# chrhansk/sleqp

Measured on AMD Instinct MI355X. Metric: KKT factor+solve/sec (numeric refactor + 1 solve with device-controlled refinement, inputs resident in HBM), higher is better.
Workload: dtype f64; 1 GPU; banded_n1e5_m5e4; n=100000, m=50000, N=150000, nnz_J=1000000, nnz_tril_K=1100000, nnz_L=11646539, nnz_L_stored=12226637, supernodes=569, etree_levels=10, refine_steps=1, hip_graphs=5, solves_per_factor=1, parallelism=single

## Files before the change

include/hipfact.h:

```cpp
#ifndef HIPFACT_H
#define HIPFACT_H

#include <stddef.h>
#include <stdint.h>

#ifdef __cplusplus
extern "C" {
#endif

#define HIPFACT_VERSION "0.1.0"

enum
{
  HIPFACT_OK         = 0,
  HIPFACT_EINVAL     = -1,
  HIPFACT_EDEVICE    = -2,
  HIPFACT_ESINGULAR  = -3,
  HIPFACT_ENOMEM     = -4,
  HIPFACT_ESTATE     = -5,
  HIPFACT_EINTERNAL  = -6
};

typedef struct hipfact_handle hipfact_handle;

// ... 151 lines not shown
  HIPFACT_LSQR_TIME      = 3,
  HIPFACT_LSQR_ZERO      = 4
};

typedef struct hipfact_lsqr_info
{
  double time_limit;
  int iterations;
  int status;
  int timed_out;
  double phi_bar;
} hipfact_lsqr_info;

int hipfact_lsqr_solve(hipfact_handle* h, const hipfact_lsqr_op* op, const double* rhs, double rel_tol,
                       double trust_radius, double eps, int max_iter, double* step, hipfact_lsqr_info* info);

int hipfact_tridiag_tr(int k, const double* delta, const double* gamma, double gamma0, double radius, double* h,
                       double* lambda);


int hipfact_set_option(hipfact_handle* h, const char* name, double value);

int hipfact_get_info(const hipfact_handle* h, const char* name, double* value);

int hipfact_debug_copy(hipfact_handle* h, const char* name, void* out, size_t bytes);

int hipfact_debug_pool_selftest(int callers, int rounds);

int hipfact_debug_place_rows(int m, const int* Ar_ptr, long long fill_bytes, int classes, long long* bounds, int* classes_out,
                             int* grid_out, int* blocks);
int hipfact_debug_place_items(int nfronts, const int* counts, int classes, int* order, int* lost);

int hipfact_debug_multi_slices(int u, int slice_rows, int* tile_bounds , int cap);

int hipfact_debug_extra_rule(int nblocks, int npasses, const double* dn, const double* zn, int pass_cap, int* applied,
                             int* status, double* ferr, double* rho);
int hipfact_debug_multi_extra_schedule(int ncols, int nblocks, int npasses, const double* dn, const double* zn,
                                       int pass_cap, unsigned int* open_mask, hipfact_extra_info* info);
int hipfact_debug_condest_dense(int N, const double* A, long long ld, hipfact_cond_info* info,
                                double* witness , int* history , int cap);
int hipfact_debug_condest_recorded(int N, int nrecords, const double* records, hipfact_cond_info* info);
enum {
  HIPFACT_CADENCE_FACTOR = 0,
  HIPFACT_CADENCE_SOLVE = 1,
  HIPFACT_CADENCE_VERDICT = 2,
  HIPFACT_CADENCE_JUDGE = 3,
  HIPFACT_CADENCE_RESET = 4,
  HIPFACT_CADENCE_SET_STEPS = 5,
  HIPFACT_CADENCE_SET_CHECK_EVERY = 6,
  HIPFACT_CADENCE_SET_CHECK_BACKOFF = 7,
  HIPFACT_CADENCE_SAVE = 8,
  HIPFACT_CADENCE_RESTORE = 9,
  HIPFACT_CADENCE_DEVICE_RESIDUAL = 10,
  HIPFACT_CADENCE_EVENT_WIDTH = 8,
  HIPFACT_CADENCE_ROW_WIDTH = 20
};
int hipfact_debug_refine_cadence(const int* knobs , int nevents, const double* events, long long* rows);
double hipfact_debug_dd_residual(int nterms, const double* k, const double* z, double b, int lanes);


typedef struct hipfact_plan hipfact_plan;
int hipfact_plan_create(int N, const int* colptr, const int* rowidx, const double* vals ,
                        hipfact_plan** out);
void hipfact_plan_free(hipfact_plan** plan);
const char* hipfact_plan_error(const hipfact_plan* plan);
int hipfact_plan_array(const hipfact_plan* plan, const char* name, const void** data, int64_t* len,
// ... 9 lines not shown
```

sleqp_amd/_lib.py:

```python
from __future__ import annotations

import ctypes as C
import os

_HERE = os.path.dirname(os.path.abspath(__file__))
LIB_PATH = os.environ.get("HIPFACT_LIBRARY") or os.path.join(_HERE, "csrc", "libhipfact.so")

HIPFACT_OK = 0
ERRORS = {
    -1: "HIPFACT_EINVAL",
    -2: "HIPFACT_EDEVICE",
    -3: "HIPFACT_ESINGULAR",
    -4: "HIPFACT_ENOMEM",
    -5: "HIPFACT_ESTATE",
    -6: "HIPFACT_EINTERNAL",
}

SYMBOLS = [
    "hipfact_create", "hipfact_free", "hipfact_retain", "hipfact_last_error", "hipfact_last_warning", "hipfact_set_matrix", "hipfact_solve_sparse",
    "hipfact_solve_dense", "hipfact_solution", "hipfact_solution_view", "hipfact_condition", "hipfact_refactor_device",
    "hipfact_solve_device", "hipfact_solve_device_multi", "hipfact_solve_multi",
    "hipfact_condition_estimate", "hipfact_debug_condest_dense", "hipfact_debug_condest_recorded",
    "hipfact_solve_device_extra", "hipfact_solve_extra", "hipfact_residual_device", "hipfact_debug_extra_rule", "hipfact_debug_dd_residual",
    "hipfact_solve_device_multi_extra", "hipfact_solve_multi_extra", "hipfact_residual_device_multi", "hipfact_debug_multi_extra_schedule",
    "hipfact_solution_device", "hipfact_synchronize", "hipfact_check", "hipfact_stream",
    "hipfact_assemble_kkt", "hipfact_reduced_matrix", "hipfact_spmat_create", "hipfact_spmat_update_values", "hipfact_spmat_free",
    "hipfact_spmat_mult_vec", "hipfact_spmat_mult_vec_trans", "hipfact_spmat_mult_vec_sym",
    "hipfact_spmat_mult_device", "hipfact_steihaug_solve", "hipfact_tr_solve", "hipfact_tr_solve_ex", "hipfact_lsqr_solve", "hipfact_tridiag_tr", "hipfact_set_option", "hipfact_get_info", "hipfact_debug_copy", "hipfact_debug_pool_selftest",
    "hipfact_debug_place_rows", "hipfact_debug_place_items", "hipfact_debug_multi_slices", "hipfact_debug_refine_cadence", "hipfact_plan_create",
    "hipfact_plan_free", "hipfact_plan_error", "hipfact_plan_array", "hipfact_plan_scalar",
]

_lib = None


class HipfactError(RuntimeError):
    def __init__(self, code: int, message: str):
        super().__init__(f"{ERRORS.get(code, code)}: {message}")
        self.code = code


def load() -> C.CDLL:
    global _lib
    if _lib is not None:
        return _lib
    if not os.path.exists(LIB_PATH):
        raise ImportError(
            f"{LIB_PATH} not found: build the HIP extension first "
            "(python -c 'import __graft_entry__ as g; g.build()' or make -C sleqp_amd/csrc)")
    lib = C.CDLL(LIB_PATH)
    vp, ci, cd = C.c_void_p, C.c_int, C.c_double
    lib.hipfact_create.argtypes = [C.POINTER(vp), ci]
    lib.hipfact_free.argtypes = [C.POINTER(vp)]
    lib.hipfact_retain.argtypes = [vp]
    lib.hipfact_last_error.argtypes = [vp]
    lib.hipfact_last_error.restype = C.c_char_p
    lib.hipfact_last_warning.argtypes = [vp]
    lib.hipfact_last_warning.restype = C.c_char_p
    lib.hipfact_set_matrix.argtypes = [vp, ci, vp, vp, vp]
    lib.hipfact_solve_sparse.argtypes = [vp, ci, ci, vp, vp]
    lib.hipfact_solve_dense.argtypes = [vp, vp]
    lib.hipfact_solution.argtypes = [vp, vp, ci, ci]
# ... 17 lines not shown
        lib.hipfact_residual_device_multi.argtypes = [vp, ci, vp, ll, vp, ll, vp, ll, ci]
        lib.hipfact_debug_multi_extra_schedule.argtypes = [ci, ci, ci, vp, vp, ci, vp, vp]
    if hasattr(lib, "hipfact_condition_estimate"):
        lib.hipfact_condition_estimate.argtypes = [vp, ci, vp, vp]
        lib.hipfact_debug_condest_dense.argtypes = [ci, vp, C.c_longlong, vp, vp, vp, ci]
        lib.hipfact_debug_condest_recorded.argtypes = [ci, ci, vp, vp]
    lib.hipfact_solution_device.argtypes = [vp, C.POINTER(vp)]
    lib.hipfact_synchronize.argtypes = [vp]
    lib.hipfact_check.argtypes = [vp]
    lib.hipfact_stream.argtypes = [vp, C.POINTER(vp)]
    lib.hipfact_assemble_kkt.argtypes = [vp, ci, ci, vp, vp, vp, vp, vp, ci, C.POINTER(ci), vp, vp, vp]
    lib.hipfact_reduced_matrix.argtypes = [vp, C.POINTER(ci), vp, vp, vp]
    lib.hipfact_spmat_create.argtypes = [vp, ci, ci, vp, vp, vp, C.POINTER(vp)]
    lib.hipfact_spmat_update_values.argtypes = [vp, vp]
    lib.hipfact_spmat_free.argtypes = [C.POINTER(vp)]
    lib.hipfact_spmat_mult_vec.argtypes = [vp, vp, vp]
    lib.hipfact_spmat_mult_vec_trans.argtypes = [vp, vp, vp]
    lib.hipfact_spmat_mult_vec_sym.argtypes = [vp, vp, vp]
    lib.hipfact_spmat_mult_device.argtypes = [vp, ci, vp, vp]
    lib.hipfact_steihaug_solve.argtypes = [vp, vp, vp, cd, cd, ci, vp, C.POINTER(cd), C.POINTER(ci)]
    lib.hipfact_tr_solve.argtypes = [vp, ci, vp, vp, vp, vp, cd, cd, ci, vp, C.POINTER(cd), C.POINTER(ci)]
    lib.hipfact_tr_solve_ex.argtypes = [vp, ci, vp, vp, vp, vp, cd, cd, ci, vp, C.POINTER(cd), C.POINTER(ci), vp]
    lib.hipfact_lsqr_solve.argtypes = [vp, vp, vp, cd, cd, cd, ci, vp, vp]
    lib.hipfact_tridiag_tr.argtypes = [ci, vp, vp, cd, cd, vp, C.POINTER(cd)]
    lib.hipfact_set_option.argtypes = [vp, C.c_char_p, cd]
    lib.hipfact_debug_copy.argtypes = [vp, C.c_char_p, vp, C.c_size_t]
    lib.hipfact_debug_pool_selftest.argtypes = [ci, ci]
    lib.hipfact_get_info.argtypes = [vp, C.c_char_p, C.POINTER(cd)]
    if hasattr(lib, "hipfact_debug_place_items"):
        lib.hipfact_debug_place_rows.argtypes = [ci, vp, C.c_longlong, ci, vp, C.POINTER(ci), C.POINTER(ci), vp]
        lib.hipfact_debug_place_items.argtypes = [ci, vp, ci, vp, vp]
    if hasattr(lib, "hipfact_debug_multi_slices"):
        lib.hipfact_debug_multi_slices.argtypes = [ci, ci, vp, ci]
    if hasattr(lib, "hipfact_debug_refine_cadence"):
        lib.hipfact_debug_refine_cadence.argtypes = [vp, ci, vp, vp]
    lib.hipfact_plan_create.argtypes = [ci, vp, vp, vp, C.POINTER(vp)]
    lib.hipfact_plan_free.argtypes = [C.POINTER(vp)]
    lib.hipfact_plan_error.argtypes = [vp]
    lib.hipfact_plan_error.restype = C.c_char_p
    lib.hipfact_plan_array.argtypes = [vp, C.c_char_p, C.POINTER(vp), C.POINTER(C.c_int64), C.POINTER(ci)]
    lib.hipfact_plan_scalar.argtypes = [vp, C.c_char_p, C.POINTER(cd)]
    for name in SYMBOLS:
        if not hasattr(lib, name) and not os.environ.get("HIPFACT_LIBRARY"):
            raise ImportError(f"{LIB_PATH} lacks {name}: rebuild it (make -C sleqp_amd/csrc)")
    lib.hipfact_plan_free.restype = None
    _lib = lib
    return lib


def kernel_sources_sha16() -> str:
    import glob
    import hashlib

    d = os.path.join(os.path.dirname(os.path.abspath(__file__)), "csrc")
    h = hashlib.sha256()
    for name in sorted(glob.glob(os.path.join(d, "*.hip")) + glob.glob(os.path.join(d, "*.inc")) + glob.glob(os.path.join(d, "*.h"))):
        h.update(os.path.basename(name).encode())
        h.update(open(name, "rb").read())
    return h.hexdigest()[:16]
```

sleqp_amd/csrc/abi_options.inc:

```
enum OptionEffect {
  FX_NONE,
  FX_GRAPHS,
  FX_GRAPHS_IF_CHANGED,
  FX_PLANS,
  FX_PLANS_IF_CHANGED,
};
struct OptionRow {
  const char* name;
  const char* env;
  OptionEffect effect;
  int (*set)(hipfact_handle* h, double v);
  const char* doc;
};
#define OPT_STORE(field, conv)                 \
  [](hipfact_handle* h, double v) -> int {     \
    const auto x = (conv);                     \
    const bool changed = h->field != x;        \
    h->field = x;                              \
    return changed;                            \
  }
static const OptionRow kOptions[] = {
    {"refine_steps", "HIPFACT_REFINE", FX_GRAPHS,
     [](hipfact_handle* h, double v) -> int {
       h->refine_steps = std::max(0, (int)v);
// ... 135 lines not shown
     },
     "1: K is analysed exactly as given - no row dictionary, unit rows of active bounds stay in the structure (what hipfact_reduced_matrix needs)"},
    {"assemble_superset", nullptr, FX_NONE, OPT_STORE(assemble_superset, v != 0.0),
     "0: hipfact_assemble_kkt analyses every working set on its own rows (no superset plan)"},
    {"plan_cache", nullptr, FX_NONE,
     [](hipfact_handle* h, double v) -> int {
       h->plan_cache_max = std::max(0, (int)v);
       while ((int)h->cache.size() > h->plan_cache_max) h->cache.pop_back();
       return 1;
     },
     "inactive plan states kept (LRU); 0: one pattern at a time"},
    {"profile", nullptr, FX_NONE,
     [](hipfact_handle* h, double v) -> int {
       if (h->prof.on) prof_collect(h);
       if (v < 0)
         for (int c = 0; c < PC_COUNT; ++c) h->prof.ms[c] = 0, h->prof.max_ms[c] = 0, h->prof.cnt[c] = 0;
       h->prof.tagged.clear();
       h->prof.on = v > 0;
       return 1;
     },
     "event-time every kernel class; value < 0 resets the counters"},
    {"ordering", nullptr, FX_PLANS, OPT_STORE(prm.ordering, (int)v),
     "0 nested dissection + AMD leaves (default), 1 AMD on the whole graph, 2 natural"},
    {"max_children", nullptr, FX_PLANS, OPT_STORE(prm.max_children, (int)v),
     "relaxed amalgamation keeps fronts at this many children (default 4 = what the pull extend-add takes in one block)"},
    {"force_generic", nullptr, FX_PLANS, OPT_STORE(prm.force_generic, v != 0.0),
     "1: no saddle-point structure detection, static 1 x 1 pivots on K as given (symmetric positive definite input: the PSD shim)"},
    {"dense_mode", nullptr, FX_PLANS, OPT_STORE(prm.dense_mode, std::min(2, std::max(0, (int)v))),
     "1: late elimination inside the tree (default), 2: low-rank correction, 0: off"},
    {nullptr, "HIPFACT_DATAFLOW_RETRY", FX_NONE, OPT_STORE(df_retry_every, std::max(0, (int)v)), nullptr},
    {nullptr, "HIPFACT_CHECK_LAUNCHES", FX_NONE, OPT_STORE(check_launches, v != 0.0), nullptr},
    {nullptr, "HIPFACT_SOL_SPLIT", FX_NONE, OPT_STORE(sol_split, v != 0.0), nullptr},
    {nullptr, "HIPFACT_IDX64", FX_NONE, OPT_STORE(idx64, v != 0.0), nullptr},
    {nullptr, "HIPFACT_XCD_CLASSES", FX_NONE, OPT_STORE(xcd_classes, std::max(1, std::min(XCD_CLASSES_MAX, (int)v))), nullptr},
    {nullptr, "HIPFACT_RESID_FROM_X", FX_NONE, OPT_STORE(resid_from_x, std::max(0, std::min(3, (int)v))), nullptr},
};
#undef OPT_STORE

static void options_from_environment(hipfact_handle* h) {
  for (const OptionRow& row : kOptions)
    if (const char* s = row.env ? getenv(row.env) : nullptr) (void)row.set(h, (double)atoi(s));
}

int hipfact_set_option(hipfact_handle* h, const char* name, double value) {
  if (!h || !name) return HIPFACT_EINVAL;
  {
    bool known = false;
    const int rc = multi_set_option(h, name, value, known);
    if (known) return rc;
  }
  {
    bool known = false;
    const int rc = condest_set_option(h, name, value, known);
    if (known) return rc;
  }
  for (const OptionRow& row : kOptions) {
    if (!row.name || strcmp(name, row.name)) continue;
    const int changed = row.set(h, value);
    if (changed < 0) return changed;
    if (row.effect == FX_GRAPHS || (row.effect == FX_GRAPHS_IF_CHANGED && changed)) drop_graphs(h);
    if (row.effect == FX_PLANS || (row.effect == FX_PLANS_IF_CHANGED && changed)) invalidate_plans(h);
    return HIPFACT_OK;
  }
  h->error = std::string("unknown option: ") + name;
  return HIPFACT_EINVAL;
}

int hipfact_debug_copy(hipfact_handle* h, const char* name, void* out, size_t bytes) {
  int rc = enter(h);
  if (rc) return rc;
  if (!name || !out) return HIPFACT_EINVAL;
  auto host_copy = [&](const auto& v) {
    if (bytes > v.size() * sizeof(v[0])) {
      h->error = "hipfact_debug_copy: unknown buffer or size";
      return HIPFACT_EINVAL;
    }
    if (bytes) memcpy(out, v.data(), bytes);
    return HIPFACT_OK;
  };
  const Plan& P = h->plan;
  if (!strcmp(name, "perm")) return host_copy(P.perm);
  if (!strcmp(name, "sn_c0")) return host_copy(P.sn_c0);
  if (!strcmp(name, "sn_r")) return host_copy(P.sn_r);
  if (!strcmp(name, "sn_rowptr")) return host_copy(P.sn_rowptr);
  if (!strcmp(name, "sn_rows")) return host_copy(P.sn_rows);
  if (!strcmp(name, "sn_Loff")) return host_copy(P.sn_Loff);
  if (!strcmp(name, "late_cols")) return host_copy(P.late_cols);
  if (!strcmp(name, "sn_level")) return host_copy(P.sn_level);
  if (!strcmp(name, "dense_cols")) return host_copy(P.dense_cols);
  if (!strcmp(name, "cond_history")) return host_copy(h->cond_history);
  const DevBuf* b = nullptr;
  if (!strcmp(name, "L")) b = &h->d_L;
  else if (!strcmp(name, "U")) b = &h->d_U;
  else if (!strcmp(name, "SPf")) b = &h->d_SPf;
  else if (!strcmp(name, "sitems")) b = &h->d_sitems;
  else if (!strcmp(name, "y")) b = &h->d_y;
  else if (!strcmp(name, "xhat")) b = &h->d_xhat;
  else if (!strcmp(name, "ysol")) b = &h->d_ysol;
  else if (!strcmp(name, "uvec")) b = &h->d_uvec;
  else if (!strcmp(name, "dscale")) b = &h->d_dscale;
  else if (!strcmp(name, "Kval")) b = &h->d_Kval;
  else if (!strcmp(name, "res")) b = &h->d_res;
  else if (!strcmp(name, "norms")) b = &h->d_norms;
  else if (!strcmp(name, "mY")) b = &h->d_mY;
  if (!strcmp(name, "cond_d")) {
    const size_t N = (size_t)h->N_ext, off = (2 * COND_T + 3) * N * sizeof(double);
    if (!h->d_cblk.p || bytes > N * sizeof(double)) {
      h->error = "hipfact_debug_copy: unknown buffer or size";
      return HIPFACT_EINVAL;
    }
    HCHECK(h, hipStreamSynchronize(h->stream));
    HCHECK(h, hipMemcpy(out, h->d_cblk.as<char>() + off, bytes, hipMemcpyDeviceToHost));
    return HIPFACT_OK;
  }
  if (!b || !b->p || bytes > b->bytes) {
    h->error = "hipfact_debug_copy: unknown buffer or size";
    return HIPFACT_EINVAL;
  }
  HCHECK(h, hipStreamSynchronize(h->stream));
  HCHECK(h, hipMemcpy(out, b->p, bytes, hipMemcpyDeviceToHost));
  return HIPFACT_OK;
}

int hipfact_debug_place_rows(int m, const int* Ar_ptr, long long fill_bytes, int classes, long long* bounds, int* classes_out,
                             int* grid_out, int* blocks) {
  if (m < 0 || (m > 0 && !Ar_ptr) || fill_bytes < 0 || classes < 1 || classes > XCD_CLASSES_MAX || !bounds || !classes_out ||
      !grid_out || !blocks)
    return HIPFACT_EINVAL;
  ClassBounds cb;
  *grid_out = place_rows(m, Ar_ptr, (size_t)fill_bytes, classes, cb);
  *classes_out = cb.C;
  for (int g = 0; g <= cb.C; ++g) bounds[g] = cb.b[g];
  for (int g = 0; g < cb.C; ++g) class_row_blocks(cb, g, FB / RL, blocks[2 * g], blocks[2 * g + 1]);
  return HIPFACT_OK;
}
int hipfact_debug_place_items(int nfronts, const int* counts, int classes, int* order, int* lost) {
  if (nfronts < 0 || (nfronts > 0 && !counts) || classes < 1 || classes > XCD_CLASSES_MAX) return HIPFACT_EINVAL;
  long long total = 0;
  for (int f = 0; f < nfronts; ++f) {
    if (counts[f] < 0) return HIPFACT_EINVAL;
    total += counts[f];
  }
  if (total >= (1LL << 31) || (total > 0 && (!order || !lost))) return HIPFACT_EINVAL;
  std::vector<int> o, l;
  deal_items(std::vector<int>(counts, counts + nfronts), classes, o, &l);
  for (size_t i = 0; i < o.size(); ++i) {
    order[i] = o[i];
    lost[i] = l[i];
  }
  return HIPFACT_OK;
}

int hipfact_debug_multi_slices(int u, int slice_rows, int* tile_bounds, int cap) {
  if (u < 0 || !multi_slice_rows_valid(slice_rows)) return HIPFACT_EINVAL;
  const int ns = multi_nslice(u, slice_rows);
  if (tile_bounds && ns <= cap)
    for (int k = 0; k <= ns; ++k) tile_bounds[k] = multi_slice_tile(u, ns, k);
  return ns;
}

int hipfact_debug_refine_cadence(const int* knobs, int nevents, const double* events, long long* rows) {
  using namespace hipfact;
  if (!knobs || nevents < 0 || (nevents > 0 && (!events || !rows))) return HIPFACT_EINVAL;
  for (int q = 0; q < 7; ++q)
    if (knobs[q] < 0 || ((q == 1 || q >= 5) && knobs[q] > 1) || (q >= 2 && q <= 4 && knobs[q] < 1)) return HIPFACT_EINVAL;
  CadenceKnobs k{knobs[0], knobs[1] != 0, knobs[2], knobs[3], knobs[4], knobs[5] != 0, knobs[6] != 0};
  FactorCadence f;
  PlanCadence p;
  SolveCadence s;
  LiveCadence l;
  Cadence cad{f, p, s, l};
  SavedCadence saved{};
  bool have_saved = false;
  for (int e = 0; e < nevents; ++e) {
    const double* ev = events + (size_t)e * HIPFACT_CADENCE_EVENT_WIDTH;
    for (int q = 0; q < 6; ++q)
      if (!(std::fabs(ev[q]) < (double)(1 << 30)) || ev[q] != std::floor(ev[q])) return HIPFACT_EINVAL;
    const int kind = (int)ev[0], flag = (int)ev[1];
    const CtlPeek c{(int)ev[2], (int)ev[3], (int)ev[4], (int)ev[5], ev[6], ev[7]};
    const bool yes_no = flag == 0 || flag == 1;
    SolveDecision d{false, false, false, 0, 0};
    switch (kind) {
      case HIPFACT_CADENCE_FACTOR:
// ... 117 lines not shown
  INFO("nlevels", P.nlevels) INFO("nprod", P.nprod) INFO("L_bytes", P.L_size * 8.0) INFO("U_bytes", P.U_size * 8.0)
  INFO("analysis_s", P.t_total) INFO("order_s", P.t_order) INFO("symbolic_s", P.t_symbolic)
  INFO("num_perturbed", h->num_perturbed) INFO("static_pivot_runs", h->static_pivot_runs) INFO("static_pivot_shift", h->reg_delta)
  INFO("num_zero_pivots", h->info_host[INFO_ZERO_PIVOT]) INFO("num_neg_pivots", h->info_host[INFO_NEG_PIVOT])
  INFO("cache_hits", h->cache_hits) INFO("plan_swaps", h->plan_swaps) INFO("plans_cached", h->cache.size())
  INFO("no_dataflow", h->no_dataflow) INFO("dataflow_fallbacks", h->dataflow_fallbacks) INFO("turn_waits", (double)h->turn_waits) INFO("dataflow_rearmed", h->dataflow_rearmed) INFO("fused_solve", h->fused_solve) INFO("spanel_folded", h->sp_folded) INFO("solve_items", h->n_sitems) INFO("chain_levels_fused", [&] { int c = 0; for (const LevelInfo& li : h->levels) c += li.mini_cnt > 0; return c; }()) INFO("solve_panel_bytes", h->sp_bytes) INFO("spf_bytes", (double)h->d_SPf.bytes) INFO("sitem_bytes", (double)sizeof(SolveItem)) INFO("N_internal", P.N) INFO("maps_on", h->maps_on) INFO("m_struct", h->m_struct) INFO("analyses", h->analyses) INFO("num_factor", h->num_factor) INFO("cg_device_runs", h->cg_device_runs) INFO("cg_device_fallbacks", h->cg_device_fallbacks) INFO("lz_device_runs", h->lz_device_runs) INFO("lz_device_fallbacks", h->lz_device_fallbacks) INFO("lz_device_iterations", h->lz_device_iterations) INFO("lsqr_runs", h->lsqr_runs) INFO("lsqr_iters", h->lsqr_iters) INFO("dense_columns", h->nd) INFO("late_columns", P.n_late) INFO("late_rows", P.n_late_rows) INFO("m_rows", P.saddle ? P.my : P.m) INFO("vtable_rows", h->vj->rows()) INFO("vtable_retries", h->vtable_retries) INFO("dense_fallbacks", h->dense_fallbacks) INFO("dense_probes", h->dense_probes) INFO("top_block_cols", h->tb_nT) INFO("top_block_below", h->tb_nfb) INFO("top_block_levels", h->tb_levels) INFO("top_block_items", h->tb_ntf) INFO("top_block_builds", h->tb_builds) INFO("top_block_active", h->tb_valid) INFO("superset_vtable", h->superset_vtable) INFO("exact_pattern", h->exact_pattern) INFO("spmv_stream", h->spmv_stream)
  INFO("boundary_fast", h->boundary_fast) INFO("bd_count", h->bd_count) INFO("bd_stage_us", h->bd_stage_us) INFO("bd_queue_us", h->bd_queue_us) INFO("bd_rhs_us", h->bd_rhs_us) INFO("bd_device_us", h->bd_device_us) INFO("bd_d2h_us", h->bd_d2h_us) INFO("bd_wait_us", h->bd_wait_us) INFO("bd_copyout_us", h->bd_copyout_us)
  INFO("multi_solves", h->multi_solves) INFO("multi_cols", h->multi_cols) INFO("multi_blocks", h->multi_blocks)
  INFO("multi_passes", h->multi_passes) INFO("multi_single_cols", h->multi_single_cols) INFO("multi_failed_col", h->multi_failed_col)
  INFO("multi_sliced_fronts", h->mitems_for < 0 ? 0 : h->n_mcut) INFO("multi_slice_items", h->mitems_for < 0 ? 0 : h->n_mslices) INFO("multi_slice_rows", h->multi_slice_rows)
  INFO("cond_estimates", h->cond_estimates) INFO("cond_blocks", h->cond_blocks) INFO("cond_last", h->cond_last) INFO("condition_estimate", h->condition_estimate)
  INFO("extra_solves", h->extra_solves) INFO("extra_passes", h->extra_passes) INFO("extra_last_status", h->extra_last_status)
  INFO("extra_multi_solves", h->extra_multi_solves) INFO("extra_multi_cols", h->extra_multi_cols) INFO("extra_multi_passes", h->extra_multi_passes)
  INFO("num_solve", h->num_solve) INFO("num_refined", h->solve_cad.num_refined) INFO("refine_adaptive", h->refine_adaptive)
  INFO("num_passes", h->solve_cad.num_passes) INFO("last_omega", h->last_ctl.omega) INFO("last_iters", h->last_ctl.iters)
  INFO("last_status", h->last_ctl.status) INFO("last_tol", h->last_ctl.tol) INFO("kappa_est", h->last_ctl.kappa)
  INFO("refine_inline", h->factor_cad.refine_inline) INFO("refine_tol", h->refine_tol) INFO("equilibrate", h->equilibrate)
  INFO("factor_top_level", h->ftop_level) INFO("factor_top_count", h->ftop_count) INFO("solve_timeouts", h->h_info.p ? h->h_info.as<int>()[INFO_TIMEOUT] : 0)
  INFO("top_level", 1 << 30)
  INFO("use_graph", h->use_graph) INFO("num_graphs", h->graphs.size()) INFO("max_r", P.max_r) INFO("max_w", P.max_w) INFO("refine_steps", h->refine_steps)
  INFO("schur_flops_max_level", h->schur_flops_max)
  INFO("chain_pairs", h->n_pairs)
  INFO("xupd_fused", h->xupd_fused ? 1 : 0)
  INFO("rhs_in_tree", h->last_rhs_in_tree) INFO("xupd_in_tree", h->last_xupd_in_tree) INFO("xupd_blocks_launched", h->last_xupd_blocks)
  INFO("solve_sliced_fronts", h->n_sliced) INFO("solve_resorted_levels", h->n_resorted) INFO("tree_solve", tree_solve(h))
  INFO("refine_check_every", h->refine_check_every) INFO("refine_check_interval", h->solve_cad.check_interval_now) INFO("num_checked", h->solve_cad.num_checked)
  INFO("device", h->device) INFO("nnzM", P.Mi.size()) INFO("nnzA", P.Ar_src.size())
  INFO("rows_total", P.sn_rows.size()) INFO("ent_fused", h->ent_fused) INFO("ent_split", h->ent_split)
  INFO("rows_fused", h->rows_fused) INFO("rows_split", h->rows_split)
  INFO("long_row_segments", h->n_rseg) INFO("row_scale_blocks", row_scale_in_sequence(h) ? h->rs_grid : 0)
  INFO("arena_fill_bytes", arena_fill_bytes(P))
  INFO("resid_blocks", resid_blocks(P)) INFO("resid_from_x", resid_from_x(h)) INFO("resid_queued_from_x", h->resid_queued_from_x) INFO("resid_queued_full", h->resid_queued_full)
  INFO("xcd_classes", h->xcd_classes) INFO("dealt_multi_item_fronts", h->dealt_multi) INFO("long_prod_segments", h->n_lprod)
  INFO("long_col_segments", h->n_cseg) INFO("idx32", h->idx32) INFO("prod_packed", h->prod_packed)
  INFO("active_bounds", h->maps_on ? h->n_bounds : 0)
  INFO("values_in_place",
       h->have_plan && (!h->from_jacobian || (virtual_current(h) && h->vj->identity))) INFO("inactive_rows", h->maps_on ? h->n_inactive : 0)
#undef INFO
  return HIPFACT_EINVAL;
}
```

sleqp_amd/csrc/hipfact.hip:

```cpp
#include <hip/hip_runtime.h>

#include <dlfcn.h>

#include <algorithm>
#include <atomic>
#include <chrono>
#include <cmath>
#include <cstdio>
#include <cstdlib>
#include <cstring>
#include <memory>
#include <new>
#include <string>
#include <condition_variable>
#include <functional>
#include <mutex>
#include <thread>
#include <unordered_map>
#include <vector>

#include "../../include/hipfact.h"
#include "device_types.h"
#include "plan.h"
#include "tridiag_tr.h"

#include "kernel_types.h"
#include "kernels_decl.h"
#include "xcd_place.h"
#include "multi_slices.h"
#include "refine_cadence.h"
#include "condest_rule.h"
#include "dd_arith.h"

#include "runtime_types.inc"
#include "runtime_plan.inc"
#include "runtime_queue.inc"
#include "runtime_multi.inc"
#include "runtime_extra.inc"
#include "runtime_multi_extra.inc"
#include "runtime_condest.inc"

extern "C" {
#include "abi_core.inc"
#include "abi_multi.inc"
#include "abi_extra.inc"
#include "abi_multi_extra.inc"
#include "abi_condest.inc"
#include "abi_working_set.inc"
#include "abi_krylov.inc"
#include "abi_options.inc"
}
```

sleqp_amd/csrc/kernels_factor.hip:

```cpp
#include <hip/hip_runtime.h>

#include "device_types.h"
#include "kernel_types.h"

namespace hipfact {
#include "kernels_common.inc"
#include "kernels_mvals.inc"
#include "kernels_front_pivot.inc"
#include "kernels_front_update.inc"
#include "kernels_front_fused.inc"
#include "kernels_solve_panels.inc"
#include "kernels_factor_top.inc"
}

namespace hipfact {
#define INST_MVALS(IDX, PK)                                                                                          \
  template __global__ void k_mvals_prod<IDX, PK>(long long, const IDX*, const int*, const int*, const IDX*, const double*, \
                                                double*, int, const LongProd*,                                       \
                                                double*, unsigned int*);
INST_MVALS(unsigned int, true)
INST_MVALS(unsigned int, false)
INST_MVALS(long long, true)
INST_MVALS(long long, false)
#undef INST_MVALS
#define INST_FRONT(CH)                                                                                              \
  template __global__ void k_front_pivot<CH>(const FrontItem*, double*, double*, int*, const int*, const int*,     \
                                             const PullDesc*, int);                                                 \
  template __global__ void k_front_panel<CH>(const FrontItem*, double*, double*, const int*, const int*,           \
                                             const PullDesc*, int);                                                 \
  template __global__ void k_front_schur<CH>(const FrontItem*, double*, double*, const int*, const int*,           \
                                             const PullDesc*, int);
INST_FRONT(true)
INST_FRONT(false)
#undef INST_FRONT
}

// ... 12 lines not shown
```

sleqp_amd/csrc/kernels_front_update.inc:

```
template <bool X_IN_LDS, bool RECIP = false>
__device__ __forceinline__ void dev_panel_solve(const FrontCtx& c, int blk, int blk_stride, const PullCtx& pc,
                                                const int* invl) {
  const int wave = threadIdx.x >> 6;
  const int RB = 16 * (blockDim.x >> 6);
  for (int R0 = c.w + RB * blk + 16 * wave; R0 < c.r; R0 += RB * blk_stride) {
    double pv[8][4];
    int cis[MAXCH];
    dev_panel_rows_load(c, R0, pc, pv, cis);
    dev_panel_rows_finish<X_IN_LDS, RECIP>(c, R0, pc, invl, pv, cis);
  }
}

constexpr int KC = 32;
constexpr int SCB = 64;
__device__ __forceinline__ void schur_tile_gather(const PullCtx& pc, const int* invs, int i0, int j0, int li, int lk,
                                                  double (&uv)[2][2][4]) {
#pragma unroll
  for (int ch = 0; ch < MAXCH; ++ch)
    if (ch < pc.n) {
      const double* __restrict__ Uc = pc.Uc[ch];
      const int uc = pc.uc[ch];
      const int* iv = invs + 128 * ch;
      int ci[2], cj[2][4];
#pragma unroll
// ... 354 lines not shown
      J = t - a * (a + 1) / 2;
    } else {
      I = ntc + (t - head) / ntc;
      J = (t - head) % ntc;
    }
    ij = (int)((I << 16) | J);
  } else if (compact) {
    const long long nt = (c.u + 63) / 64;
    long long t = blockIdx.x, jb = 0;
    for (;; ++jb) {
      const long long j0 = jb * SCB, bw = min((long long)SCB, nt - j0), rows = nt - j0;
      const long long cnt = bw * (bw + 1) / 2 + (rows - bw) * bw;
      if (t < cnt) break;
      t -= cnt;
    }
    const long long j0 = jb * SCB, bw = min((long long)SCB, nt - j0), head = bw * (bw + 1) / 2;
    long long I, J;
    if (t < head) {
      long long a = (long long)((sqrt(8.0 * (double)t + 1.0) - 1.0) * 0.5);
      while (a * (a + 1) / 2 > t) --a;
      while ((a + 1) * (a + 2) / 2 <= t) ++a;
      I = j0 + a;
      J = j0 + (t - a * (a + 1) / 2);
    } else {
      I = j0 + bw + (t - head) / bw;
      J = j0 + (t - head) % bw;
    }
    ij = (int)((I << 16) | J);
  }
  dev_schur_tile<false, CHAIN>(c, c.A, c.A + 64 * KC, ij >> 16, ij & 0xffff, S.nchild == 0, pc, threadIdx.x, nullptr, 0,
                               nullptr, PullMore{more, U, inv, rel});
}


__global__ __launch_bounds__(FB, 3) void k_front_schur_pair(const FrontItem* __restrict__ items, double* __restrict__ L,
                                                             double* __restrict__ U, PairDesc D) {
  extern __shared__ __attribute__((aligned(16))) double lds[];
  const FrontItem& S = items[0];
  const FrontCtx c = make_ctx(S, L, U, lds);
  const int tid = threadIdx.x, lane = tid & 63, wave = tid >> 6;
  const int li = lane & 15, lk = lane >> 4;
  const int u = c.u;
  double* SI = c.A;
  double* SJ = c.A + 64 * KC;
  int I, J;
  {
    const long long nt = (u + 63) / 64;
    long long t = blockIdx.x, jb = 0;
    for (;; ++jb) {
      const long long j0 = jb * SCB, bw = min((long long)SCB, nt - j0), rows = nt - j0;
      const long long cnt = bw * (bw + 1) / 2 + (rows - bw) * bw;
      if (t < cnt) break;
      t -= cnt;
    }
    const long long j0 = jb * SCB, bw = min((long long)SCB, nt - j0), head = bw * (bw + 1) / 2;
    if (t < head) {
      long long a = (long long)((sqrt(8.0 * (double)t + 1.0) - 1.0) * 0.5);
      while (a * (a + 1) / 2 > t) --a;
      while ((a + 1) * (a + 2) / 2 <= t) ++a;
      I = (int)(j0 + a);
      J = (int)(j0 + (t - a * (a + 1) / 2));
    } else {
      I = (int)(j0 + bw + (t - head) / bw);
      J = (int)(j0 + (t - head) % bw);
    }
  }
// ... 102 lines not shown
```

sleqp_amd/csrc/runtime_plan.inc:

```

static void prof_begin(hipfact_handle* h, int cls) {
  Prof& p = h->prof;
  if (!p.on) return;
  if (p.used + 2 > p.ev.size()) {
    hipEvent_t a, b;
    if (hipEventCreate(&a) != hipSuccess || hipEventCreate(&b) != hipSuccess) return;
    p.ev.push_back(a);
    p.ev.push_back(b);
  }
  p.cls.resize(p.ev.size() / 2);
  p.fl.resize(p.ev.size() / 2);
  p.cls[p.used / 2] = cls;
  p.fl[p.used / 2] = p.next_fl;
  p.next_fl = 0.0;
  (void)hipEventRecord(p.ev[p.used], h->stream);
}
static void prof_end(hipfact_handle* h) {
  Prof& p = h->prof;
  if (!p.on || p.used + 2 > p.ev.size()) return;
  (void)hipEventRecord(p.ev[p.used + 1], h->stream);
  p.used += 2;
}
static void prof_collect(hipfact_handle* h) {
  Prof& p = h->prof;
// ... 340 lines not shown
        const long long u = P.sn_r[s] - (P.sn_c0[s + 1] - P.sn_c0[s]), nt = (u + 63) / 64;
        if (pair_role[s] == 1) {
          const int par = P.sn_parent[s];
          const long long ntc = std::min(nt, (long long)((sn[par].w + 63) / 64));
          li.compactD = true;
          li.pair = 1;
          fitems.push_back(item(s, (int)(-(ntc + 1))));
          li.nD = (int)(ntc * (ntc + 1) / 2 + (nt - ntc) * ntc);
          const double cc = 64.0 * (double)ntc;
          li.pair_flops_done = 2.0 * sn[s].w * ((double)u * cc - 0.5 * cc * cc);
          li.schur_flops_full = li.schur_flops;
          li.schur_flops = li.pair_flops_done;
        } else if (pair_role[s] == 2) {
          const int a = P.child_idx[P.child_ptr[s]], g = pair_g[s];
          li.compactD = true;
          li.pair = 2;
          fitems.push_back(item(s, -1));
          li.nD = (int)(nt * (nt + 1) / 2);
          li.pd.Loff_a = sn[a].Loff;
          li.pd.w_a = sn[a].w;
          li.pd.r_a = sn[a].r;
          li.pd.rowoff_a = sn[s].w;
          li.pd.Uoff_g = sn[g].Uoff;
          li.pd.u_g = sn[g].r - sn[g].w;
          li.pd.off_g = sn[a].w + sn[s].w;
          const LevelInfo& la = h->levels[P.sn_level[a]];
          li.schur_flops += la.schur_flops_full - la.pair_flops_done;
        } else if (nt * (nt + 1) / 2 >= 1024 && nt * (nt + 1) / 2 < (1LL << 31)) {
          li.compactD = true;
          fitems.push_back(item(s, -1));
          li.nD = (int)(nt * (nt + 1) / 2);
        }
      }
      for (int s : order) {
        if (li.compactD) break;
        const int u = P.sn_r[s] - (P.sn_c0[s + 1] - P.sn_c0[s]);
        const int nt = (u + 63) / 64;
        per_front.push_back(nt * (nt + 1) / 2);
        for (int I = 0; I < nt; ++I)
          for (int J = 0; J <= I; ++J) {
            plain.push_back(item(s, (I << 16) | J));
            ++li.nD;
          }
      }
      emit_by_class();
    }
  }
  h->ent_fused = h->ent_split = h->rows_fused = h->rows_split = 0;
  for (int l = 0; l < P.nlevels; ++l)
    for (int q = P.level_ptr[l]; q < P.level_ptr[l + 1]; ++q) {
      const int s = P.level_sn[q];
      const double w = P.sn_c0[s + 1] - P.sn_c0[s], r = P.sn_r[s];
      const double ent = w * r - w * (w - 1) / 2;
      (h->levels[l].split ? h->ent_split : h->ent_fused) += ent;
      (h->levels[l].split ? h->rows_split : h->rows_fused) += r;
    }
  if ((rc = upload(h, h->d_items, items))) return rc;
  if ((rc = upload(h, h->d_fitems, fitems))) return rc;
  auto slice_rows = [&](int w2) {
    const int fwd = 1024 / ((w2 + SOLVE_PREFETCH - 1) / SOLVE_PREFETCH);
    const int bwd = SOLVE_PREFETCH * std::max(1, 1024 / w2);
    return std::max(w2 + 16, std::min({fwd, bwd, 1024}));
  };
  std::vector<int> it_front, it_sl, it_nsl, it_a0, it_a1, first_item(ns, 0);
  std::vector<int> solve_order(P.level_sn.begin(), P.level_sn.begin() + ns);
  if (h->solve_sorted)
    for (int l = 0; l < P.nlevels; ++l)
      std::stable_sort(solve_order.begin() + P.level_ptr[l], solve_order.begin() + P.level_ptr[l + 1], [&](int a, int b) {
        return (long long)sn[a].r * sn[a].w > (long long)sn[b].r * sn[b].w;
      });
  h->n_resorted = 0;
// ... 659 lines not shown
```

sleqp_amd/csrc/runtime_queue.inc:

```
struct TurnState {
  std::mutex mu;
  hipEvent_t last = nullptr;
  hipfact_handle* owner = nullptr;
  std::atomic<int> live{0};
};
static TurnState g_turn[16];
static hipfact_handle* g_trace_handles[8] = {nullptr};
struct Turn {
  hipfact_handle* h;
  bool counted = false, held = false;
  explicit Turn(hipfact_handle* h_) : h(h_) {
    if (h->capturing) return;
    counted = true;
    if (h->turn_depth++ > 0) return;
    TurnState& T = g_turn[h->device & 15];
    static const bool off = getenv("HIPFACT_NO_TURNS") != nullptr;
    if (off || T.live.load(std::memory_order_acquire) <= 1 || !h->ev_turn) return;
    T.mu.lock();
    held = true;
    if (T.last && T.owner != h) {
      (void)hipStreamWaitEvent(h->stream, T.last, 0);
      h->turn_waits++;
    }
  }
// ... 37 lines not shown
static inline bool diag_inactive_needed(const hipfact_handle* h) {
  const Plan& P = h->plan;
  return P.saddle && P.m > 0 && ((h->maps_on && h->n_inactive > 0) || P.n_late > 0);
}
static inline bool row_scale_in_sequence(const hipfact_handle* h) {
  const Plan& P = h->plan;
  return P.saddle && P.n > 0 && P.m > 0;
}
static inline int resid_from_x(const hipfact_handle* h) {
  const Plan& P = h->plan;
  return (P.saddle && P.n > 0 && P.m > 0 && h->nd == 0 && P.n_late == 0 && h->refine_steps > 0) ? h->resid_from_x : 0;
}
static inline bool dataflow_factor(const hipfact_handle* h) { return h->debug_phases == 15 && !h->no_dataflow; }
static inline bool tree_solve(const hipfact_handle* h) { return h->fused_solve && !h->no_dataflow; }
static inline bool tree_delivers_verdict(const hipfact_handle* h) { return tree_solve(h) && h->plan.m > 0 && h->plan.saddle; }
static inline bool graph_route(const hipfact_handle* h) { return h->use_graph && !h->prof.on && h->debug_phases == 15; }
static inline const int* cmap_or_null(const hipfact_handle* h) { return (h->maps_on || h->plan.n_late > 0) ? h->d_cmap.as<int>() : nullptr; }
static inline bool masked_rows(const hipfact_handle* h) { return h->nd > 0 || h->plan.n_late > 0; }
static inline size_t arena_fill_bytes(const Plan& P) {
  return (size_t)P.L_size * sizeof(double) + (size_t)4 * P.nsuper * sizeof(int);
}
static inline int row_scale_grid(long long m, size_t fill_bytes) {
  const long long nz16 = (long long)((fill_bytes + 15) / 16);
  const int for_fill = (int)std::min<long long>(2048, std::max<long long>(1, nz16 / (FB * 8)));
  return std::max(nblocks(m * 16), for_fill);
}
static int place_rows(int m, const int* Ar_ptr, size_t fill_bytes, int classes, ClassBounds& cb) {
  return place_ranges((long long)m, FB / RL, Ar_ptr, LONG_ROW, classes, row_scale_grid(m, fill_bytes), (long long)((fill_bytes + 15) / 16), cb);
}
static void place_front_end(hipfact_handle* h) {
  const Plan& P = h->plan;
  h->rs_grid = place_rows(P.m, P.Ar_ptr.data(), arena_fill_bytes(P), h->xcd_classes, h->rs_place);
}
template <bool CH>
static void launch_schur(hipfact_handle* h, const LevelInfo& li, int pull) {
  h->prof.next_fl = li.schur_flops;
  if (li.nD <= 0) return;
  const FrontItem* fit = h->d_fitems.as<FrontItem>() + li.itD;
  if (li.pair == 2)
    LAUNCH(PC_FACTOR_D, k_front_schur_pair, dim3(li.nD), dim3(FB), li.lds_schur, fit, h->d_L.as<double>(),
           h->d_U.as<double>(), li.pd);
  else
    LAUNCH(PC_FACTOR_D, k_front_schur<CH>, dim3(li.nD), dim3(FB), li.lds_schur, fit, h->d_L.as<double>(),
           h->d_U.as<double>(), h->d_inv.as<int>(), h->d_rel.as<int>(), h->d_pullx.as<PullDesc>(), pull);
}
static int factor_enqueue(hipfact_handle* h) {
  Turn turn(h);
  const Plan& P = h->plan;
  hipStream_t st = h->stream;
  const size_t fill_bytes = arena_fill_bytes(P);
  const bool fill_rides = row_scale_in_sequence(h);
  if (!fill_rides) {
    HCHECK(h, hipMemsetAsync(h->d_info.p, 0, INFO_BYTES, st));
    if (P.L_size > 0 && fill_bytes > 0) {
      prof_begin(h, PC_MEMSET);
      HCHECK(h, hipMemsetAsync(h->d_L.p, 0, fill_bytes, st));
      prof_end(h);
    }
  }
  const long long nM = (long long)P.Mi.size();
  const int* vmap = h->maps_on ? h->d_vmap.as<int>() : nullptr;
  double* kprod = h->maps_on ? h->d_Kprod.as<double>() : h->d_Ksc.as<double>();
  if (fill_rides) {
    {
      const long long nz16 = (long long)((fill_bytes + 15) / 16);
      const bool masked = masked_rows(h);
      const double* kin = h->vals_ride ? h->vals_ride : h->d_Kval.as<double>();
      if (h->n_rseg > 0)
        LAUNCH(PC_GATHER, k_long_row_norm, dim3(std::min(h->n_rseg, 4096)), dim3(FB), 0, h->n_rseg, h->d_rseg.as<LongSeg>(),
               h->d_Ar_col.as<int>(), h->d_Ar_src.as<int>(), kin, vmap,
               masked ? h->d_dmask.as<int>() : nullptr, P.n_late > 0 ? 1 : 0, h->equilibrate ? 1 : 0,
               h->d_dscale.as<double>(), h->d_segpart.as<double>(), h->d_segcnt.as<unsigned int>());
// ... 918 lines not shown
```

sleqp_amd/csrc/runtime_types.inc:

```
namespace hipfact {

struct DevBuf {
  void* p = nullptr;
  size_t bytes = 0;
  DevBuf() = default;
  DevBuf(const DevBuf&) = delete;
  DevBuf& operator=(const DevBuf&) = delete;
  DevBuf(DevBuf&& o) noexcept : p(o.p), bytes(o.bytes) {
    o.p = nullptr;
    o.bytes = 0;
  }
  DevBuf& operator=(DevBuf&& o) noexcept {
    if (this != &o) {
      release();
      p = o.p;
      bytes = o.bytes;
      o.p = nullptr;
      o.bytes = 0;
    }
    return *this;
  }
  ~DevBuf() { release(); }
  void release() {
    if (p) (void)hipFree(p);
// ... 20 lines not shown
  ~PinBuf() {
    if (p) (void)hipHostFree(p);
  }
  hipError_t ensure(size_t n) {
    if (n <= bytes) return hipSuccess;
    if (p) (void)hipHostFree(p);
    p = nullptr;
    bytes = 0;
    hipError_t e = hipHostMalloc(&p, n, hipHostMallocDefault);
    if (e == hipSuccess) bytes = n;
    return e;
  }
  template <class T>
  T* as() const {
    return static_cast<T*>(p);
  }
};

struct LevelInfo {
  int begin = 0, count = 0;
  size_t lds_factor = 0, lds_fwd = 0, lds_bwd = 0;
  bool split = false;
  bool pull = false;
  bool chain = false;
  int nparts = 1;
  long long itA = 0;
  long long itB = 0, itC = 0, itD = 0;
  int nA = 0, nC = 0, nD = 0;
  int panel_threads = 512;
  size_t lds_pivot = 0, lds_panel = 0, lds_schur = 0, lds_asm = 0, lds_solve_max = 0;
  int pair = 0;
  PairDesc pd;
  double schur_flops_full = 0.0, pair_flops_done = 0.0;
  bool compactD = false;
  double schur_flops = 0.0;
  long long mini_off = 0;
  int mini_cnt = 0;
  size_t mini_lds = 0;
};

enum ProfClass { PC_MEMSET = 0, PC_MVALS, PC_GATHER, PC_FACTOR, PC_FACTOR_A, PC_FACTOR_B, PC_FACTOR_C, PC_FACTOR_D, PC_FACTOR_T, PC_FWD, PC_BWD, PC_RHS, PC_XUPD, PC_RESID, PC_AXPY, PC_PERM, PC_SPANEL, PC_TREE, PC_COUNT };
static const char* const kProfNames[PC_COUNT] = {"memset", "mvals", "gather", "factor", "factorA", "factorB", "factorC",
                                                 "factorD", "factorT", "fwd", "bwd", "rhs", "xupd", "resid", "axpy", "perm",
                                                 "spanel", "tree"};

struct Prof {
  bool on = false;
  std::vector<hipEvent_t> ev;
  std::vector<int> cls;
  size_t used = 0;
  double ms[PC_COUNT] = {0};
  double max_ms[PC_COUNT] = {0};
  std::vector<double> fl;
  double next_fl = 0.0;
  std::vector<std::pair<double, double>> tagged;
  long cnt[PC_COUNT] = {0};
  ~Prof() {
    for (hipEvent_t e : ev) (void)hipEventDestroy(e);
  }
};

}

using namespace hipfact;

static thread_local std::string g_create_error;
// ... 182 lines not shown
  hipfact::SolveCadence solve_cad;
  hipfact::LiveCadence live_cad;
  int refine_check_every = 8;
  int refine_check_backoff = 2;
  int refine_check_max = 64;
  double pivot_ratio = 1.0;
  bool no_solve_retry = false;
  long dense_probes = 0;
  bool decide_rides = false;
  const double* vals_ride = nullptr;
  bool use_graph = true;
  bool no_dataflow = false;
  int fake_timeouts = 0;
  long dataflow_fallbacks = 0;
  int df_retry_every = 256;
  long df_retry_at = -1;
  long dataflow_rearmed = 0;
  int debug_phases = 15;
  int solve_whole_max = 48;
  bool factor_hint_peek = true;
  int top_block_breakeven = 48;
  bool chain_pairs = true;
  int n_pairs = 0;
  long long pair_extra = 0;
  double schur_flops_max = 0.0;
  bool check_launches = false, launch_reported = false;
  double* x_dot_out = nullptr;
  int x_dot_blocks = 0;
  int xupd_blocks = 256;
  bool solve_sorted = true;
  int resid_from_x = 3;
  double* x_res_out = nullptr;
  long resid_queued_from_x = 0, resid_queued_full = 0;
  int xcd_classes = 8;
  int factor_top_max = 160;
  int factor_top_levels = 1 << 20;
  int factor_top_max_u = 1024;
  int factor_top_fine = 12;
  int top_block_after = 2;
  int top_block_max = 2048;
  long tb_builds = 0;
  bool factor_top_head = true;
  int factor_top_fused = 30;
  int factor_top_fused32 = 12;
  int factor_top_fused_u = 256;
  int factor_top_post = 64;
  int panel_small_below = 0;
  int pull_max_children = 4;
  long cache_hits = 0, analyses = 0, num_factor = 0;
  int info_host[INFO_WORDS] = {0, 0, 0, 0};
  Prof prof;
  DevBuf d_info, d_norms, d_ctl;
  PinBuf h_ctl;
  void* h_ctl_dev = nullptr;
  PinBuf h_stage, h_info;
  DevBuf d_sp_idx, d_sp_val;
  PinBuf h_rhs_pin[2], h_sol_pin, h_info_pre;
  void* h_rhs_dev[2] = {nullptr, nullptr};
  void* h_sol_dev = nullptr;
  int boundary_pieces = 4;
  hipEvent_t ev_rhs[2] = {nullptr, nullptr}, ev_sol = nullptr, ev_sol_x = nullptr;
  int sol_nx = 0;
  bool sol_split = true;
  bool idx64 = false;
  bool ev_rhs_used[2] = {false, false};
  int rhs_slot = 0;
// ... 118 lines not shown
```

Baseline: 1515 factor+solve/s.

## Add leaf Schur kernel with larger 96-row MFMA tiles for split levels

Adds a new Schur-complement update kernel for split levels. It uses 96x96 tiles (NB=3) staged through LDS in 16-column chunks, with register double-buffered global loads and F64 MFMA accumulation. The plan selects it when a level has at least 256 tiles at the 64-row granularity and is neither compacted nor multi-chunk. It is on by default and can be turned off through an option. The aim is more data reuse and fewer work items per front, at the cost of more register and LDS pressure and wasted work on partial edge tiles.

After: 1535 factor+solve/s, median of 6. +1.3%, better.

```diff
diff --git a/include/hipfact.h b/include/hipfact.h
--- a/include/hipfact.h
+++ b/include/hipfact.h
@@ -207,6 +207,8 @@
 int hipfact_debug_place_items(int nfronts, const int* counts, int classes, int* order, int* lost);
 
 int hipfact_debug_multi_slices(int u, int slice_rows, int* tile_bounds , int cap);
+
+int hipfact_debug_schur_items(int u, int leaf);
 
 int hipfact_debug_extra_rule(int nblocks, int npasses, const double* dn, const double* zn, int pass_cap, int* applied,
                              int* status, double* ferr, double* rho);
diff --git a/sleqp_amd/_lib.py b/sleqp_amd/_lib.py
--- a/sleqp_amd/_lib.py
+++ b/sleqp_amd/_lib.py
@@ -27,7 +27,7 @@
     "hipfact_assemble_kkt", "hipfact_reduced_matrix", "hipfact_spmat_create", "hipfact_spmat_update_values", "hipfact_spmat_free",
     "hipfact_spmat_mult_vec", "hipfact_spmat_mult_vec_trans", "hipfact_spmat_mult_vec_sym",
     "hipfact_spmat_mult_device", "hipfact_steihaug_solve", "hipfact_tr_solve", "hipfact_tr_solve_ex", "hipfact_lsqr_solve", "hipfact_tridiag_tr", "hipfact_set_option", "hipfact_get_info", "hipfact_debug_copy", "hipfact_debug_pool_selftest",
-    "hipfact_debug_place_rows", "hipfact_debug_place_items", "hipfact_debug_multi_slices", "hipfact_debug_refine_cadence", "hipfact_plan_create",
+    "hipfact_debug_place_rows", "hipfact_debug_place_items", "hipfact_debug_multi_slices", "hipfact_debug_schur_items", "hipfact_debug_refine_cadence", "hipfact_plan_create",
     "hipfact_plan_free", "hipfact_plan_error", "hipfact_plan_array", "hipfact_plan_scalar",
 ]
 
@@ -111,6 +111,8 @@
         lib.hipfact_debug_place_items.argtypes = [ci, vp, ci, vp, vp]
     if hasattr(lib, "hipfact_debug_multi_slices"):
         lib.hipfact_debug_multi_slices.argtypes = [ci, ci, vp, ci]
+    if hasattr(lib, "hipfact_debug_schur_items"):
+        lib.hipfact_debug_schur_items.argtypes = [ci, ci]
     if hasattr(lib, "hipfact_debug_refine_cadence"):
         lib.hipfact_debug_refine_cadence.argtypes = [vp, ci, vp, vp]
     lib.hipfact_plan_create.argtypes = [ci, vp, vp, vp, C.POINTER(vp)]
diff --git a/sleqp_amd/csrc/abi_options.inc b/sleqp_amd/csrc/abi_options.inc
--- a/sleqp_amd/csrc/abi_options.inc
+++ b/sleqp_amd/csrc/abi_options.inc
@@ -191,6 +191,7 @@
     {nullptr, "HIPFACT_CHECK_LAUNCHES", FX_NONE, OPT_STORE(check_launches, v != 0.0), nullptr},
     {nullptr, "HIPFACT_SOL_SPLIT", FX_NONE, OPT_STORE(sol_split, v != 0.0), nullptr},
     {nullptr, "HIPFACT_IDX64", FX_NONE, OPT_STORE(idx64, v != 0.0), nullptr},
+    {nullptr, "HIPFACT_LEAF_SCHUR", FX_NONE, OPT_STORE(leaf_schur, v != 0.0), nullptr},
     {nullptr, "HIPFACT_XCD_CLASSES", FX_NONE, OPT_STORE(xcd_classes, std::max(1, std::min(XCD_CLASSES_MAX, (int)v))), nullptr},
     {nullptr, "HIPFACT_RESID_FROM_X", FX_NONE, OPT_STORE(resid_from_x, std::max(0, std::min(3, (int)v))), nullptr},
 };
@@ -244,6 +245,7 @@
   if (!strcmp(name, "sn_rowptr")) return host_copy(P.sn_rowptr);
   if (!strcmp(name, "sn_rows")) return host_copy(P.sn_rows);
   if (!strcmp(name, "sn_Loff")) return host_copy(P.sn_Loff);
+  if (!strcmp(name, "sn_Uoff")) return host_copy(P.sn_Uoff);
   if (!strcmp(name, "late_cols")) return host_copy(P.late_cols);
   if (!strcmp(name, "sn_level")) return host_copy(P.sn_level);
   if (!strcmp(name, "dense_cols")) return host_copy(P.dense_cols);
@@ -308,6 +310,11 @@
     lost[i] = l[i];
   }
   return HIPFACT_OK;
+}
+
+int hipfact_debug_schur_items(int u, int leaf) {
+  if (u < 0 || leaf < 0 || leaf > 1) return HIPFACT_EINVAL;
+  return schur_items(u, leaf ? LEAF_EDGE : 64);
 }
 
 int hipfact_debug_multi_slices(int u, int slice_rows, int* tile_bounds, int cap) {
@@ -491,6 +498,14 @@
   INFO("arena_fill_bytes", arena_fill_bytes(P))
   INFO("resid_blocks", resid_blocks(P)) INFO("resid_from_x", resid_from_x(h)) INFO("resid_queued_from_x", h->resid_queued_from_x) INFO("resid_queued_full", h->resid_queued_full)
   INFO("xcd_classes", h->xcd_classes) INFO("dealt_multi_item_fronts", h->dealt_multi) INFO("long_prod_segments", h->n_lprod)
+  if (!strcmp(name, "leaf_schur_levels") || !strcmp(name, "leaf_schur_items")) {
+    int levels;
+    long long items;
+    leaf_schur_counts(h, levels, items);
+    *value = !strcmp(name, "leaf_schur_levels") ? (double)levels : (double)items;
+    return HIPFACT_OK;
+  }
+  INFO("leaf_schur", h->leaf_schur)
   INFO("long_col_segments", h->n_cseg) INFO("idx32", h->idx32) INFO("prod_packed", h->prod_packed)
   INFO("active_bounds", h->maps_on ? h->n_bounds : 0)
   INFO("values_in_place",
diff --git a/sleqp_amd/csrc/hipfact.hip b/sleqp_amd/csrc/hipfact.hip
--- a/sleqp_amd/csrc/hipfact.hip
+++ b/sleqp_amd/csrc/hipfact.hip
@@ -27,6 +27,7 @@
 #include "kernel_types.h"
 #include "kernels_decl.h"
 #include "xcd_place.h"
+#include "leaf_schur.h"
 #include "multi_slices.h"
 #include "refine_cadence.h"
 #include "condest_rule.h"
diff --git a/sleqp_amd/csrc/kernels_factor.hip b/sleqp_amd/csrc/kernels_factor.hip
--- a/sleqp_amd/csrc/kernels_factor.hip
+++ b/sleqp_amd/csrc/kernels_factor.hip
@@ -2,6 +2,7 @@
 
 #include "device_types.h"
 #include "kernel_types.h"
+#include "leaf_schur.h"
 
 namespace hipfact {
 #include "kernels_common.inc"
diff --git a/sleqp_amd/csrc/kernels_front_update.inc b/sleqp_amd/csrc/kernels_front_update.inc
--- a/sleqp_amd/csrc/kernels_front_update.inc
+++ b/sleqp_amd/csrc/kernels_front_update.inc
@@ -410,6 +410,122 @@
                                nullptr, PullMore{more, U, inv, rel});
 }
 
+template <int NB, int KCH>
+__device__ __forceinline__ void dev_leaf_schur_tile(const FrontCtx& c, int I, int J) {
+  constexpr int E = 32 * NB, HB = 16 * NB, LS = E + 16;
+  constexpr int NV = E * KCH / FB;
+  static_assert(E * KCH % FB == 0 && KCH % 4 == 0, "a chunk is a whole number of entries per thread and of pivot groups");
+  const int tid = threadIdx.x, lane = tid & 63;
+  const int wave = __builtin_amdgcn_readfirstlane(tid >> 6);
+  const int li = lane & 15, lk = lane >> 4;
+  const int w = c.w, r = c.r, u = c.u;
+  double* SI = c.A;
+  double* SJ = c.A + KCH * LS;
+  const bool diag = I == J;
+  const int wi = wave & 1, wj = wave >> 1;
+  const int i0 = E * I + HB * wi, j0 = E * J + HB * wj;
+  unsigned bm = 0;
+#pragma unroll
+  for (int x = 0; x < NB; ++x)
+#pragma unroll
+    for (int y = 0; y < NB; ++y)
+      if (i0 + 16 * y < u && j0 + 16 * x < u && i0 + 16 * y + 15 >= j0 + 16 * x) bm |= 1u << (NB * x + y);
+  d4_t acc[NB][NB];
+#pragma unroll
+  for (int x = 0; x < NB; ++x)
+#pragma unroll
+    for (int y = 0; y < NB; ++y) acc[x][y] = (d4_t){0.0, 0.0, 0.0, 0.0};
+  constexpr int NH = NV / 2, KH = FB * NH / E;
+  static_assert(NV % 2 == 0 && FB * NH % E == 0 && 2 * KH == KCH, "the two halves of a thread's entries share their rows");
+  int ek[NH], loff[NH];
+  unsigned goff[NH];
+  bool iok[NH], jok[NH];
+#pragma unroll
+  for (int t = 0; t < NH; ++t) {
+    const int e = tid + FB * t, k = e / E, row = e - E * k;
+    ek[t] = k;
+    goff[t] = (unsigned)(row + k * r);
+    loff[t] = k * LS + row;
+    iok[t] = E * I + row < u;
+    jok[t] = E * J + row < u;
+  }
+  const double* __restrict__ pI = c.P + w + E * I;
+  const double* __restrict__ pJ = c.P + w + E * J;
+  auto request = [&](int n, double (&vi)[NV], double (&vj)[NV]) {
+    const int kcn = min(KCH, w - n * KCH);
+#pragma unroll
+    for (int h = 0; h < 2; ++h) {
+      const double* __restrict__ qI = pI + (long long)(n * KCH + KH * h) * r;
+      const double* __restrict__ qJ = pJ + (long long)(n * KCH + KH * h) * r;
+#pragma unroll
+      for (int t = 0; t < NH; ++t) {
+        vi[t + NH * h] = (iok[t] && ek[t] + KH * h < kcn) ? qI[goff[t]] : 0.0;
+        if (!diag) vj[t + NH * h] = (jok[t] && ek[t] + KH * h < kcn) ? qJ[goff[t]] : 0.0;
+      }
+    }
+  };
+  auto chunk = [&](int n, const double (&vi)[NV], const double (&vj)[NV]) {
+    const int kc0 = n * KCH, kcn = min(KCH, w - kc0);
+    __syncthreads();
+#pragma unroll
+    for (int h = 0; h < 2; ++h)
+#pragma unroll
+      for (int t = 0; t < NH; ++t) {
+        SI[loff[t] + KH * h * LS] = vi[t + NH * h];
+        SJ[loff[t] + KH * h * LS] = (diag ? vi[t + NH * h] : vj[t + NH * h]) * c.dd[kc0 + ek[t] + KH * h];
+      }
+    __syncthreads();
+    if (bm) {
+      const int ng = (kcn + 3) >> 2;
+      for (int g = 0; g < ng; ++g) {
+        const int ko = (4 * g + lk) * LS + li;
+        double a[NB], b[NB];
+#pragma unroll
+        for (int x = 0; x < NB; ++x) a[x] = SJ[ko + HB * wj + 16 * x];
+#pragma unroll
+        for (int y = 0; y < NB; ++y) b[y] = SI[ko + HB * wi + 16 * y];
+#pragma unroll
+        for (int x = 0; x < NB; ++x)
+#pragma unroll
+          for (int y = 0; y < NB; ++y)
+            if (bm & (1u << (NB * x + y))) acc[x][y] = MFMA_F64(a[x], b[y], acc[x][y]);
+      }
+    }
+  };
+  {
+    double ai[NV], aj[NV], bi[NV], bj[NV];
+    const int nc = (w + KCH - 1) / KCH;
+    request(0, ai, aj);
+    for (int n = 0; n < nc; n += 2) {
+      if (n + 1 < nc) request(n + 1, bi, bj);
+      chunk(n, ai, aj);
+      if (n + 2 < nc) request(n + 2, ai, aj);
+      if (n + 1 < nc) chunk(n + 1, bi, bj);
+    }
+  }
+#pragma unroll
+  for (int x = 0; x < NB; ++x)
+#pragma unroll
+    for (int y = 0; y < NB; ++y)
+      if (bm & (1u << (NB * x + y))) {
+        const int i = i0 + 16 * y + li;
+#pragma unroll
+        for (int q = 0; q < 4; ++q) {
+          const int j = j0 + 16 * x + lk + 4 * q;
+          if (i < u && j < u && i >= j) c.Us[i + (long long)j * u] = 0.0 - acc[x][y][q];
+        }
+      }
+}
+
+__global__ __launch_bounds__(FB, 3) void k_leaf_schur(const FrontItem* __restrict__ items, double* __restrict__ L,
+                                                       double* __restrict__ U) {
+  extern __shared__ __attribute__((aligned(16))) double lds[];
+  const FrontItem& S = items[blockIdx.x];
+  const FrontCtx c = make_ctx(S, L, U, lds);
+  for (int t = threadIdx.x; t < c.wp; t += FB) c.dd[t] = (t < c.w) ? c.P[t + (long long)t * c.r] : 0.0;
+  dev_leaf_schur_tile<LEAF_NB, LEAF_KCH>(c, S.part >> 16, S.part & 0xffff);
+}
+
 
 __global__ __launch_bounds__(FB, 3) void k_front_schur_pair(const FrontItem* __restrict__ items, double* __restrict__ L,
                                                              double* __restrict__ U, PairDesc D) {
diff --git a/sleqp_amd/csrc/leaf_schur.h b/sleqp_amd/csrc/leaf_schur.h
--- /dev/null
+++ b/sleqp_amd/csrc/leaf_schur.h
@@ -0,0 +1,20 @@
+#pragma once
+#include <cstddef>
+
+namespace hipfact {
+
+constexpr int LEAF_NB = 3;
+constexpr int LEAF_EDGE = 32 * LEAF_NB;
+constexpr int LEAF_KCH = 16;
+constexpr int LEAF_LS = LEAF_EDGE + 16;
+
+constexpr int LEAF_MIN_TILES = 256;
+
+inline int schur_tile_rows(int u, int edge) { return (u + edge - 1) / edge; }
+inline int schur_items(int u, int edge) {
+  const int nt = schur_tile_rows(u, edge);
+  return nt * (nt + 1) / 2;
+}
+inline size_t leaf_schur_lds(size_t wp) { return (wp + 2 * (size_t)LEAF_LS * LEAF_KCH) * sizeof(double); }
+
+}
diff --git a/sleqp_amd/csrc/runtime_plan.inc b/sleqp_amd/csrc/runtime_plan.inc
--- a/sleqp_amd/csrc/runtime_plan.inc
+++ b/sleqp_amd/csrc/runtime_plan.inc
@@ -396,11 +396,16 @@
           li.nD = (int)(nt * (nt + 1) / 2);
         }
       }
+      long long tiles64 = 0;
+      for (int s : order) tiles64 += schur_items(P.sn_r[s] - (P.sn_c0[s + 1] - P.sn_c0[s]), 64);
+      li.leaf = mch == 0 && !li.compactD && h->leaf_schur && tiles64 >= LEAF_MIN_TILES;
+      if (li.leaf) li.lds_schur = leaf_schur_lds(wp);
+      const int edge = li.leaf ? LEAF_EDGE : 64;
       for (int s : order) {
         if (li.compactD) break;
         const int u = P.sn_r[s] - (P.sn_c0[s + 1] - P.sn_c0[s]);
-        const int nt = (u + 63) / 64;
-        per_front.push_back(nt * (nt + 1) / 2);
+        const int nt = schur_tile_rows(u, edge);
+        per_front.push_back(schur_items(u, edge));
         for (int I = 0; I < nt; ++I)
           for (int J = 0; J <= I; ++J) {
             plain.push_back(item(s, (I << 16) | J));
diff --git a/sleqp_amd/csrc/runtime_queue.inc b/sleqp_amd/csrc/runtime_queue.inc
--- a/sleqp_amd/csrc/runtime_queue.inc
+++ b/sleqp_amd/csrc/runtime_queue.inc
@@ -93,12 +93,24 @@
   const Plan& P = h->plan;
   h->rs_grid = place_rows(P.m, P.Ar_ptr.data(), arena_fill_bytes(P), h->xcd_classes, h->rs_place);
 }
+static inline void leaf_schur_counts(const hipfact_handle* h, int& levels, long long& items) {
+  levels = 0;
+  items = 0;
+  const int below = dataflow_factor(h) ? std::min(h->ftop_level, h->plan.nlevels) : h->plan.nlevels;
+  for (int l = 0; l < below && l < (int)h->levels.size(); ++l)
+    if (h->levels[l].split && h->levels[l].leaf && h->levels[l].nD > 0) {
+      ++levels;
+      items += h->levels[l].nD;
+    }
+}
 template <bool CH>
 static void launch_schur(hipfact_handle* h, const LevelInfo& li, int pull) {
   h->prof.next_fl = li.schur_flops;
   if (li.nD <= 0) return;
   const FrontItem* fit = h->d_fitems.as<FrontItem>() + li.itD;
-  if (li.pair == 2)
+  if (li.leaf)
+    LAUNCH(PC_FACTOR_D, k_leaf_schur, dim3(li.nD), dim3(FB), li.lds_schur, fit, h->d_L.as<double>(), h->d_U.as<double>());
+  else if (li.pair == 2)
     LAUNCH(PC_FACTOR_D, k_front_schur_pair, dim3(li.nD), dim3(FB), li.lds_schur, fit, h->d_L.as<double>(),
            h->d_U.as<double>(), li.pd);
   else
diff --git a/sleqp_amd/csrc/runtime_types.inc b/sleqp_amd/csrc/runtime_types.inc
--- a/sleqp_amd/csrc/runtime_types.inc
+++ b/sleqp_amd/csrc/runtime_types.inc
@@ -76,6 +76,7 @@
   int pair = 0;
   PairDesc pd;
   double schur_flops_full = 0.0, pair_flops_done = 0.0;
+  bool leaf = false;
   bool compactD = false;
   double schur_flops = 0.0;
   long long mini_off = 0;
@@ -324,6 +325,7 @@
   int resid_from_x = 3;
   double* x_res_out = nullptr;
   long resid_queued_from_x = 0, resid_queued_full = 0;
+  bool leaf_schur = true;
   int xcd_classes = 8;
   int factor_top_max = 160;
   int factor_top_levels = 1 << 20;
```
